# zhenghao2519/Beyond-Fixed-Forms

Hardware: AMD Instinct MI355X
Metric: scenes/sec (2D->3D projection+refinement), 200k pts x 300 views (higher is better)
Workload: dtype f64

## Files before the change

### beyond_fixed_forms_amd/_lib.py

```python
from __future__ import annotations

import ctypes
import os
import time
from ctypes import c_double, c_float, c_int32, c_int64, c_void_p

import torch

_HERE = os.path.dirname(os.path.abspath(__file__))
LIB_PATH = os.environ.get("BFF_HIP_LIB") or os.path.join(_HERE, "lib", "libbff_hip.so")
CSRC_DIR = os.path.join(_HERE, "csrc")

_P, _I, _L, _D, _F = c_void_p, c_int32, c_int64, c_double, c_float

SIGNATURES = {
    "bff_rle_to_maskbits": [_P, _P, _P, _P, _I, _L, _I, _P, _P, _P],
    "bff_rle_to_labels": [_P, _P, _P, _P, _I, _L, _I, _P, _P, _P, _P],
    "bff_mask_row_directory": [_P, _P, _P, _I, _I, _I, _P, _P],
    "bff_project_views_lookup": [_P, _L, _L, _P, _P, _I, _P, _I, _I, _I, _P, _I, _I, _D, _P, _P, _P, _P, _P, _I, _P, _P, _P, _P, _P, _L, _L, _P, _P, _P, _P],
    "bff_project_views_cached": [_L, _I, _P, _I, _I, _P, _P, _P, _P, _P, _P, _P, _P, _I, _P, _P, _P, _P, _P, _L, _L, _P, _P, _P, _P],
    "bff_visibility_table": [_P, _L, _L, _P, _P, _I, _P, _I, _I, _I, _I, _I, _D, _P, _P, _P, _P, _L, _P, _I, _P],
    "bff_visibility_sorted": [_P, _P, _P, _L, _L, _I, _I, _I, _P, _P, _P, _P, _P, _P],
    "bff_project_views_runs": [_L, _I, _P, _I, _I, _P, _P, _P, _P, _P, _P, _P, _P, _I, _P, _P, _P, _P, _P, _L, _L, _P, _P, _P, _P],
    "bff_masks2d_count": [_P, _I, _L, _P, _P, _P],
    "bff_masks2d_runs": [_P, _I, _L, _P, _P, _P, _P],
    "bff_project_views": [_P, _L, _L, _P, _P, _I, _P, _P, _I, _I, _D, _P, _P, _P, _I, _P, _P, _P, _P, _P, _L, _L, _P, _P, _P, _P, _P],
    "bff_depth_tile_u16": [_P, _I, _I, _I, _P, _I, _P],
    "bff_project_views_u16": [_P, _L, _L, _P, _P, _I, _P, _I, _I, _I, _P, _I, _I, _D, _P, _P, _P, _I, _P, _P, _P, _P, _P, _L, _L, _P, _P, _P, _P, _P],
    "bff_point_tile_bounds": [_P, _L, _L, _P, _P],
    "bff_count_viewed": [_P, _L, _L, _P, _P, _I, _P, _I, _I, _I, _P, _I, _I, _D, _I, _P, _P, _P],
    "bff_render_depth_u16": [_P, _L, _L, _P, _P, _I, _I, _I, _I, _I, _I, _P, _P, _P, _P],
    "bff_render_splat_depth_u16": [_P, _L, _L, _P, _P, _I, _I, _I, _I, _I, _D, _I, _P, _P, _P, _P],
    "bff_point_labels": [_P, _I, _L, _L, _P, _P, _P],
    "bff_render_labels_u16": [_P, _L, _L, _P, _P, _P, _I, _I, _I, _I, _I, _D, _I, _P, _P, _P, _P, _P],
    "bff_label_runs_count": [_P, _I, _I, _I, _I, _I, _I, _P, _P, _P],
    "bff_label_runs_emit": [_P, _I, _I, _I, _I, _I, _I, _P, _L, _P, _P, _P, _P],
    "bff_render_mesh_depth_u16": [_P, _L, _L, _P, _L, _P, _P, _I, _I, _I, _I, _I, _I, _P, _P, _P],
    "bff_render_mesh_depth_clip_u16": [_P, _L, _L, _P, _L, _P, _P, _I, _I, _I, _I, _I, _D, _I, _P, _P, _P],
# ... 392 lines not shown
def sweep_runs_ok(n_points):
    return bool(load().bff_sweep_runs_ok(n_points))


def project_views_runs(n_points, depth_index, height, width, vis, vis_sorted, run_start, run_end, mask_run_offs,
                       view_mask_offs, word_bits, frame_mask, frame_rowbase, frame_nmask, frame_flags, rows, masked_count,
                       viewed_count, chunk_mask):
    call("bff_project_views_runs", n_points, depth_index.shape[0], _ptr(depth_index, i32), height, width,
         _ptr(vis[0], i64), _ptr(vis_sorted[0], i32), _ptr(vis_sorted[1], i32), _ptr(vis_sorted[2], i32),
         _ptr(run_start, i32), _ptr(run_end, i32), _ptr(mask_run_offs, i32), _ptr(view_mask_offs, i32), word_bits,
         _ptr(frame_mask, i32), _ptr(frame_rowbase, i32), _ptr(frame_nmask, i32), _ptr(frame_flags, i32), _ptr(rows, i64),
         0 if rows is None else rows.shape[0], (n_points + 63) // 64, _ptr(chunk_mask, i64), _ptr(masked_count, i32),
         _ptr(viewed_count, i32))


def count_viewed(xyz_soa, n_points, inv_pose, cam_intr, depth, depth_index, height, width, depth_thresh, viewed_count,
                 tile_bounds=None, depth_size=None, frames_per_block=None):
    k = (c_double * 9)(*[float(v) for v in cam_intr.reshape(-1)])
    if depth.dtype == torch.int16 or depth_size is not None:
        hs, ws = (depth_size if depth_size is not None else depth.shape[1:3])
        layout = 0 if depth_size is None else (2 if depth.dtype == f32 else 1)
    else:
        hs, ws, layout = 0, 0, -1
        if depth.dtype != f32:
            raise TypeError(f"expected float32 depth images, got {depth.dtype}")
    if frames_per_block is None:
        frames_per_block = int(os.environ.get("BFF_VIEWED_TILE", "0"))
    call("bff_count_viewed", _ptr(xyz_soa, f64), n_points, xyz_soa.shape[1], _ptr(inv_pose, f64), ctypes.cast(k, c_void_p),
         inv_pose.shape[0], _ptr(depth), int(hs), int(ws), layout, _ptr(depth_index, i32), height, width,
         float(depth_thresh), int(frames_per_block), _ptr(viewed_count, i32), _ptr(tile_bounds, f64))
# ... 566 lines not shown
```

### beyond_fixed_forms_amd/csrc/common.h

```cpp
#pragma once

#include <hip/hip_runtime.h>

#include <cstdarg>
#include <cstdint>
#include <cstdio>

#include "bff_hip.h"

namespace bff {

constexpr int kWave = 64;
constexpr int kCW = 8;

char *err_buf();

inline int fail(int code, const char *fmt, ...) {
    va_list ap;
    va_start(ap, fmt);
    vsnprintf(err_buf(), 512, fmt, ap);
    va_end(ap);
    return code;
}

// ... 10 lines not shown
int &scratch_prezeroed();
inline hipError_t zero_async(void *p, size_t bytes, hipStream_t st)
{
    return scratch_prezeroed() ? hipSuccess : hipMemsetAsync(p, 0, bytes, st);
}

#define BFF_REQUIRE(cond, ...) \
    do { if (!(cond)) return ::bff::fail(BFF_E_ARG, __VA_ARGS__); } while (0)
#define BFF_LIMIT(cond, ...) \
    do { if (!(cond)) return ::bff::fail(BFF_E_LIMIT, __VA_ARGS__); } while (0)

__device__ __forceinline__ int lane_id() { return threadIdx.x & (kWave - 1); }

__device__ __forceinline__ int popc64(uint64_t v) { return __popcll(v); }

__device__ __forceinline__ void rle_word_edges(const uint64_t *row, int64_t w, int64_t nw, uint64_t &starts,
                                               uint64_t &ends)
{
    const uint64_t cur = w < nw ? row[w] : 0;
    const uint64_t prev_bit = w ? (row[w - 1] >> 63) : 0;
    const uint64_t shifted = (cur << 1) | prev_bit;
    starts = cur & ~shifted;
    ends = ~cur & shifted;
}

}
```

### beyond_fixed_forms_amd/csrc/merge.hip

```cpp
#include <hip/hip_ext.h>

#include <cstdlib>

#include "rows.h"

static thread_local hipEvent_t g_merge_start = nullptr, g_merge_stop = nullptr;

namespace bff {

constexpr int kBins = 64;

__device__ __forceinline__ int64_t heavy_signature(uint64_t heavy)
{
    uint32_t key = 0;
#pragma unroll
    for (int s = 0; s < 5; ++s) {
        int b = 63;
        if (heavy) { b = __ffsll((unsigned long long)heavy) - 1; heavy &= heavy - 1; }
        key = (key << 6) | (uint32_t)b;
    }
    return (int64_t)key;
}

__global__ __launch_bounds__(256) void row_stats_kernel(const uint64_t *__restrict__ rows, int64_t nw, int mw,
                                                         int bin_words, int32_t *__restrict__ area,
                                                         int32_t *__restrict__ mean_word,
                                                         uint64_t *__restrict__ cmask, uint32_t *__restrict__ hist,
                                                         int64_t *__restrict__ signature, uint16_t *__restrict__ cpop)
{
    extern __shared__ uint64_t s_cm[];
    __shared__ int part[4];
    __shared__ unsigned long long psum[4];
    __shared__ uint32_t s_hist[kBins];
    const int r = blockIdx.x, tid = threadIdx.x;
    const uint64_t *row = rows + (int64_t)r * nw;
    for (int i = tid; i < mw; i += 256) s_cm[i] = 0;
    if (tid < kBins) s_hist[tid] = 0;
// ... 1103 lines not shown
```

### beyond_fixed_forms_amd/csrc/project.hip

```cpp
#include <algorithm>
#include <cstdlib>

#include <hip/hip_ext.h>
#include <rocprim/device/device_radix_sort.hpp>

#include "common.h"
#include "mask_rows.h"

namespace bff {

constexpr int kBlock = 256;
constexpr int kPPT = 4;
constexpr int kWordsPerBlock = (kBlock / kWave) * kPPT;
constexpr int kPtsPerBlock = kWordsPerBlock * kWave;

struct Intrinsics { double k[9]; };

struct RawDepth {
    const uint32_t *taps;
    int n_taps;
    int texel_f32;
    int64_t frame_stride;
    float scale;
};
// ... 779 lines not shown
    const int64_t t = (int64_t)blockIdx.x * kBlock + threadIdx.x;
    if (t >= (int64_t)n_slots * (H + 1)) return;
    const int s = (int)(t / (H + 1)), y = (int)(t - (int64_t)s * (H + 1));
    int64_t lo = min((int64_t)off[s * stride], n_pairs);
    int64_t hi = s + 1 < n_slots ? min((int64_t)off[(s + 1) * stride], n_pairs) : n_pairs;
    const uint32_t target = (uint32_t)y * (uint32_t)W;
    while (lo < hi) {
        const int64_t mid = lo + ((hi - lo) >> 1);
        if (spix[mid] < target) lo = mid + 1; else hi = mid;
    }
    rowstart[t] = (uint32_t)lo;
}

constexpr int kRunsDeal = 4;

__global__ __launch_bounds__(kBlock) void sweep_runs_fill_kernel(
    int n_frames, const int32_t *__restrict__ depth_index, int H, int W,
    const uint32_t *__restrict__ spix, const uint32_t *__restrict__ spt, const uint32_t *__restrict__ rowstart,
    const int32_t *__restrict__ run_start, const int32_t *__restrict__ run_end, const int32_t *__restrict__ mask_run_offs,
    const int32_t *__restrict__ view_mask_offs, const int32_t *__restrict__ frame_mask,
    const int32_t *__restrict__ frame_rowbase, const int32_t *__restrict__ frame_nmask,
    uint64_t *__restrict__ rows, int64_t nw, int n_chunks, uint64_t *__restrict__ chunk_mask, int mw)
{
    extern __shared__ uint64_t s_row[];
    const int f = blockIdx.x, m = blockIdx.y;
    const int mi = frame_mask[f];
    if (mi < 0 || m >= frame_nmask[f]) return;
    const int tid = threadIdx.x, lane = tid & 63, wave = tid >> 6;
    const int64_t row = (int64_t)frame_rowbase[f] + m;
    for (int i = tid; i < n_chunks * kCW; i += kBlock) s_row[i] = 0;
    __syncthreads();

    const int g = view_mask_offs[mi] + m;
    const int r0 = mask_run_offs[g], r1 = mask_run_offs[g + 1];
    const uint32_t *rs = rowstart + (int64_t)depth_index[f] * (H + 1);
    const int hw = H * W;
    uint32_t *bits = reinterpret_cast<uint32_t *>(s_row);
    for (int rb = r0 + wave * kWave; rb < r1; rb += kBlock) {
        const int r = rb + lane;
        uint32_t lo = 0, cnt = 0;
        if (r < r1) {
            const int start = max(run_start[r], 0), end = min(run_end[r], hw);
            if (start < end) {
                const int y = start / W, ye = (end - 1) / W;
                uint32_t lo1 = rs[y], hi1 = rs[y + 1], lo2 = rs[ye], hi2 = rs[ye + 1];
// ... 48 lines not shown
        for (int h = 0; h < kCW; h += kPPT) {
            uint64_t o = 0;
#pragma unroll
            for (int q = 0; q < kPPT; ++q) o |= v[h + q];
            if (o) {
                any = true;
#pragma unroll
                for (int q = 0; q < kPPT; ++q) {
                    const int64_t w = (int64_t)c * kCW + h + q;
                    if (w < nw) rows[row * nw + w] = v[h + q];
                }
            }
        }
        const uint64_t flags = __ballot(any);
        if (lane == 0 && flags) chunk_mask[row * mw + (c0 >> 6)] |= flags;
    }
}

constexpr int kCountBlock = 1024;
constexpr int kCountBatch = 4;
constexpr int kCountList = 4096;

__global__ __launch_bounds__(kCountBlock) void sweep_runs_count_kernel(const uint64_t *__restrict__ rows, int64_t n_rows, int64_t nw,
                                                                       const uint64_t *__restrict__ chunk_mask, int mw,
                                                                       int64_t n_points, int32_t *__restrict__ masked_count)
{
    __shared__ int s_cnt[kCW * kWave];
    __shared__ int s_list[kCountList];
    __shared__ int s_n;
    const int tid = threadIdx.x, lane = tid & 63, wave = tid >> 6;
// ... 694 lines not shown

static int64_t runs_row_bytes(int64_t n_points)
{
    return (int64_t)sizeof(uint64_t) * kCW * ceil_div(ceil_div(n_points, (int64_t)kWave), (int64_t)kCW);
}

extern "C" int32_t bff_sweep_runs_ok(int64_t n_points)
{
    const char *on = getenv("BFF_SWEEP_RUNS"), *cap = getenv("BFF_SWEEP_RUNS_LDS_BYTES");
    if (on && on[0] == '0' && on[1] == 0) return 0;
    int64_t bound = kRunsLdsMax;
    if (cap && *cap) bound = std::min<int64_t>(bound, std::max<int64_t>(0, atoll(cap)));
    return n_points > 0 && runs_row_bytes(n_points) <= bound;
}

extern "C" int bff_project_views_runs(int64_t n_points, int32_t n_frames, const int32_t *depth_index, int32_t height,
                                      int32_t width, const uint64_t *vis_mask, const uint32_t *vis_spix,
                                      const uint32_t *vis_spt, const uint32_t *vis_rowstart, const int32_t *run_start,
                                      const int32_t *run_end, const int32_t *mask_run_offs, const int32_t *view_mask_offs,
                                      int32_t word_bits, const int32_t *frame_mask, const int32_t *frame_rowbase,
                                      const int32_t *frame_nmask, const int32_t *frame_flags, uint64_t *rows, int64_t n_rows,
                                      int64_t nw, uint64_t *chunk_mask, int32_t *masked_count, int32_t *viewed_count,
                                      void *stream)
{
    if (n_points <= 0 || n_frames <= 0) return BFF_OK;
    BFF_REQUIRE(height > 0 && width > 0, "bff_project_views_runs: bad image size");
    BFF_LIMIT((int64_t)height * width < (1ll << 31), "bff_project_views_runs: image larger than 2^31 pixels");
    BFF_REQUIRE(vis_mask && vis_spix && vis_spt && vis_rowstart, "bff_project_views_runs: null table");
    BFF_REQUIRE(word_bits == 32 || word_bits == 64, "bff_project_views_runs: word_bits must be 32 or 64");
    BFF_REQUIRE(depth_index && frame_mask && frame_rowbase && frame_nmask && frame_flags && run_start && run_end &&
                mask_run_offs && view_mask_offs && rows && chunk_mask && n_rows >= 0, "bff_project_views_runs: null pointer");
    BFF_REQUIRE(nw == ceil_div(n_points, 64), "bff_project_views_runs: nw must be ceil(n_points/64)");
    const int64_t row_bytes = runs_row_bytes(n_points);
    BFF_LIMIT(row_bytes <= kRunsLdsMax, "bff_project_views_runs: an instance row exceeds 64 KB of LDS (bff_sweep_runs_ok)");
    hipStream_t st = as_stream(stream);
    const int n_chunks = (int)ceil_div(nw, kCW), mw = (int)ceil_div(n_chunks, 64);
    const hipEvent_t ev0 = g_sweep_start, ev1 = g_sweep_stop;
    g_sweep_start = g_sweep_stop = nullptr;
    const bool count = masked_count != nullptr && n_rows > 0, viewed = viewed_count != nullptr;
    hipExtLaunchKernelGGL(sweep_runs_fill_kernel, dim3((unsigned)n_frames, (unsigned)word_bits), dim3(kBlock),
        (unsigned)row_bytes, st, ev0, (count || viewed) ? nullptr : ev1, 0,
        n_frames, depth_index, height, width, vis_spix, vis_spt, vis_rowstart, run_start, run_end, mask_run_offs,
        view_mask_offs, frame_mask, frame_rowbase, frame_nmask, rows, nw, n_chunks, chunk_mask, mw);
    if (count)
        hipExtLaunchKernelGGL(sweep_runs_count_kernel, dim3((unsigned)n_chunks), dim3(kCountBlock), 0, st,
            nullptr, viewed ? nullptr : ev1, 0, rows, n_rows, nw, chunk_mask, mw, n_points, masked_count);
    if (viewed)
        hipExtLaunchKernelGGL(sweep_runs_viewed_kernel, dim3((unsigned)ceil_div(nw, kBlock / kWave)), dim3(kBlock), 0, st,
            nullptr, ev1, 0, n_frames, depth_index, frame_flags, vis_mask, bff_visibility_words(n_points), nw, n_points,
            viewed_count);
    return launched("bff_project_views_runs");
}

extern "C" int bff_visibility_sorted_bytes(int32_t n_slots, int32_t height, int64_t n_pixels, int64_t *bytes)
{
    BFF_REQUIRE(n_slots >= 0 && height >= 0 && n_pixels >= 0 && bytes, "bff_visibility_sorted_bytes: bad arguments");
    bytes[0] = (int64_t)sizeof(uint32_t) * n_pixels;
    bytes[1] = (int64_t)sizeof(uint32_t) * n_pixels;
    bytes[2] = (int64_t)sizeof(uint32_t) * n_slots * ((int64_t)height + 1);
    return BFF_OK;
}

extern "C" int bff_visibility_sorted(const uint64_t *vis_mask, const uint32_t *vis_off, const uint32_t *vis_pix,
                                     int64_t n_pixels, int64_t n_points, int32_t n_slots, int32_t height, int32_t width,
                                     uint32_t *vis_spix, uint32_t *vis_spt, uint32_t *vis_rowstart, void *temp,
                                     size_t *temp_bytes, void *stream)
// ... 177 lines not shown
```

### beyond_fixed_forms_amd/csrc/scene.hip

```cpp
#include "rows.h"

using namespace bff;

namespace {

__global__ void order_keys_kernel(const int64_t *__restrict__ sig, const int32_t *__restrict__ label_id, int n,
                                  int sig_bits, int64_t *__restrict__ keys)
{
    const int i = blockIdx.x * blockDim.x + threadIdx.x;
    if (i < n) keys[i] = ((int64_t)label_id[i] << sig_bits) | sig[i];
}

int bits_for(int n)
{
    int b = 1;
    while ((1 << b) < n && b < 31) ++b;
    return b;
}

}

#define BFF_TRY(call) do { const int rc_ = (call); if (rc_ != BFF_OK) return rc_; } while (0)

extern "C" int32_t bff_scene_header_words(int32_t s1_rows, int32_t cap)
// ... 66 lines not shown
        BFF_TRY(hand_over(ws->events[0], stream, hv));
    }
    const bool cached = lookup && sc->vis_mask && sc->vis_off && sc->vis_pix;
    const bool runs = cached && sc->vis_spix && sc->vis_spt && sc->vis_rowstart && bff_sweep_runs_ok(n) != 0;
    if (lookup && !runs) {
        BFF_REQUIRE(ws->mask_tab && ws->mask_dir, "bff_scene_project: no row directory buffers");
        BFF_TRY(bff_mask_row_directory(sc->run_start, sc->run_end, sc->mask_run_offs, n_rows, sc->height, sc->width,
                                       ws->mask_tab, ws->mask_dir, hv));
    } else if (!lookup) {
        BFF_TRY(bff_rle_to_labels(sc->run_start, sc->run_end, sc->mask_run_offs, sc->view_mask_offs, sc->n_mviews, hw,
                                  sc->word_bits, ws->labels, ws->maskbits, ws->segmap, hv));
    }
    const bool ratio = pr->filter_mode == 2;
    int32_t *const sweep_viewed = (ratio && !viewed_in) ? ws->viewed : nullptr;
    const int32_t *const viewed = ratio ? (viewed_in ? viewed_in : ws->viewed) : nullptr;
    if (runs)
        BFF_TRY(bff_project_views_runs(n, sc->n_frames, sc->depth_index, sc->height, sc->width, sc->vis_mask, sc->vis_spix,
                                       sc->vis_spt, sc->vis_rowstart, sc->run_start, sc->run_end, sc->mask_run_offs,
                                       sc->view_mask_offs, sc->word_bits, sc->frame_mask, sc->frame_rowbase, sc->frame_nmask,
                                       sc->frame_flags, ws->rows, n_rows, nw, ws->chunk_mask, ws->masked, sweep_viewed, hv));
    else if (cached)
        BFF_TRY(bff_project_views_cached(n, sc->n_frames, sc->depth_index, sc->height, sc->width, sc->vis_mask, sc->vis_off,
                                         sc->vis_pix, ws->mask_tab, ws->mask_dir, sc->run_start, sc->run_end,
                                         sc->view_mask_offs, sc->word_bits, sc->frame_mask, sc->frame_rowbase, sc->frame_nmask,
                                         sc->frame_flags, ws->rows, n_rows, nw, ws->chunk_mask, ws->masked, sweep_viewed, hv));
    else if (lookup)
        BFF_TRY(bff_project_views_lookup(sc->xyz, n, sc->n_pad, sc->inv_pose, sc->cam_intr, sc->n_frames,
                                         sc->depth_raw ? sc->depth_raw : (const void *)sc->depth, sc->depth_h, sc->depth_w,
                                         sc->depth_raw ? sc->depth_tiled : -1, sc->depth_index, sc->height, sc->width,
                                         pr->depth_thresh, ws->mask_tab, ws->mask_dir, sc->run_start, sc->run_end,
                                         sc->view_mask_offs, sc->word_bits, sc->frame_mask, sc->frame_rowbase, sc->frame_nmask,
                                         sc->frame_flags, ws->rows, n_rows, nw, ws->chunk_mask, ws->masked, sweep_viewed,
                                         sc->tile_bounds, hv));
    else if (sc->depth_raw)
        BFF_TRY(bff_project_views_u16(sc->xyz, n, sc->n_pad, sc->inv_pose, sc->cam_intr, sc->n_frames, sc->depth_raw,
// ... 24 lines not shown
        } else {
            BFF_TRY(bff_point_threshold_pairs(ws->masked, viewed, n, pr->filter_fraction,
                                              ws->pair_scratch, reinterpret_cast<float *>(hdr + BFF_HDR_THR),
                                              hdr + BFF_HDR_NUNIQUE, hdr + BFF_HDR_OVERFLOW, stream));
        }
        BFF_TRY(bff_ratio_keep(ws->masked, viewed, n, 0.0f,
                               reinterpret_cast<const float *>(hdr + BFF_HDR_THR), 1, nw, ws->keep, stream));
    } else {
        BFF_TRY(bff_ratio_keep(ws->masked, nullptr, n, 0.0f, nullptr, 0, nw, ws->keep, stream));
    }
    if (fork) {
        hipError_t ee = hipEventRecord(reinterpret_cast<hipEvent_t>(ws->aux_events[1]), as_stream(stream));
        if (ee != hipSuccess) return fail((int)ee, "bff_scene_project: aux stream: %s", hipGetErrorString(ee));
        stream = main_stream;
    }
    uint16_t *cpop = bff_merge_uses_chunk_bound(nw) ? ws->chunk_pop : nullptr;
    BFF_TRY(bff_row_stats(ws->rows, n_rows, nw, ws->area, ws->mean_word, ws->chunk_mask, 1, ws->hist, ws->sig, cpop, stream));
    {
        const int64_t *keys = ws->sig;
        int key_bits = BFF_SIGNATURE_BITS;
        if (sc->n_label_ids > 1) {
            key_bits += bits_for(sc->n_label_ids);
            order_keys_kernel<<<(unsigned)ceil_div(n_rows, 256), 256, 0, st>>>(ws->sig, sc->label_id, n_rows,
                                                                              BFF_SIGNATURE_BITS, ws->sig_keys);
            keys = ws->sig_keys;
        }
        size_t tb = ws->sort_temp_bytes;
        BFF_TRY(bff_argsort_i64(keys, ws->sig_sorted, ws->order, n_rows, key_bits, ws->sort_temp, &tb, stream));
    }
    BFF_TRY(merge_components_streams(ws->rows, n_rows, nw, ws->order, n_rows, ws->chunk_mask, ws->tile_mask, ws->hist,
                                     ws->merge_scratch, ws->area, sc->label_id, pr->iou_thres, ws->parent, 1, nullptr, nullptr,
                                     cpop, stream, hv, ws->events[2], ws->events[3]));
// ... 32 lines not shown
```

### beyond_fixed_forms_amd/projection.py

```python
from __future__ import annotations

import dataclasses
from typing import List, Optional

import numpy as np
import torch

import os

from . import _lib, pipeline
from .scene import (DEPTH_THRESH, DeviceScene, prepare_class, prepare_geometry, prepare_scene,
                    with_viewed_counts)
from .timing import merge_span, span, sweep_span


@dataclasses.dataclass
class Stage2Result:
    scene_id: str
    n_points: int
    rows: torch.Tensor
    conf: torch.Tensor
    final_class: List[str]
    groups: list
    debug: dict
# ... 126 lines not shown
def fast_path_ok(ds: DeviceScene) -> bool:
    return (ds.n_rows > 0 and ds.n_points > 0 and ds.view_mask_offs.shape[0] > 1 and ds.n_mask_frames > 0
            and ds.xyz.is_cuda and os.environ.get("BFF_NO_FAST") != "1")


@dataclasses.dataclass
class VisibilityTable:
    mask: torch.Tensor
    off: torch.Tensor
    pix: torch.Tensor
    ready: torch.cuda.Event
    streams: set
    spix: Optional[torch.Tensor] = None
    spt: Optional[torch.Tensor] = None
    rowstart: Optional[torch.Tensor] = None

    def tensors(self):
        return [t for t in (self.mask, self.off, self.pix, self.spix, self.spt, self.rowstart) if t is not None]


def vis_table_max_bytes():
    return int(float(os.environ.get("BFF_VIS_TABLE_MAX_MB", "512")) * (1 << 20))


def scene_visibility(ds: DeviceScene, depth_thresh) -> Optional[VisibilityTable]:
    if os.environ.get("BFF_VIS_TABLE", "1") == "0" or not _lib.mask_lookup_rows(ds.height, ds.width, ds.n_rows):
        return None
    owner = ds.geometry if ds.geometry is not None else ds
    tables = owner.__dict__.setdefault("_vis_tables", {})
    key = float(depth_thresh)
    tab = tables.get(key)
    if tab is None:
        tables[key] = "visited"
        return None
    if tab is False:
        return None
    raw = _lib.raw_stream()
    if tab == "visited":
        dev = ds.xyz.device
        if ds.geometry is not None:
# ... 4 lines not shown
            slots, idx = np.unique(di, return_index=True)
            first[slots] = idx
            poses = ds.inv_pose[torch.as_tensor(first).to(dev)].contiguous()
        got = _lib.visibility_table(ds.xyz, ds.n_points, poses, ds.cam_intr, ds.sweep_depth, ds.height, ds.width, key,
                                    ds.tile_bounds, depth_size=ds.depth_size, max_bytes=vis_table_max_bytes(), with_count=True)
        if got is None:
            tables[key] = False
            return None
        got, n_pairs = got[:3], got[3]
        n_slots = int(got[0].shape[0])
        total = sum(_lib.visibility_table_bytes(ds.n_points, n_slots, n_pairs)) + \
            sum(_lib.visibility_sorted_bytes(n_slots, ds.height, n_pairs))
        companion = (None, None, None)
        if _lib.sweep_runs_ok(ds.n_points) and total <= vis_table_max_bytes() and n_slots * ds.height * ds.width <= 1 << 32:
            companion = _lib.visibility_sorted(got, n_pairs, ds.n_points, ds.height, ds.width)
        ready = torch.cuda.Event()
        ready.record(torch.cuda.current_stream(dev))
        tab = tables[key] = VisibilityTable(*got, ready, {raw}, *companion)
    elif raw not in tab.streams:
        st = torch.cuda.current_stream(ds.xyz.device)
        st.wait_event(tab.ready)
        for t in tab.tensors():
            t.record_stream(st)
        tab.streams.add(raw)
    return tab


def projection_front(ds: DeviceScene, cfg, debug_out: bool = False, timers=None, stage1=None, fast=None) -> _Front:
    if fast is None:
        fast = not debug_out
    do_ratio = with_viewed_counts(cfg)
    viewed_in = ds.viewed_in if do_ratio else None
    if do_ratio and ds.geometry is not None and viewed_in is None:
        raise ValueError("a class scene needs its geometry's viewed counts for the detection-ratio filter "
                         "(prepare the geometry with with_viewed=True)")
    if fast and fast_path_ok(ds) and (stage1 is None or stage1.n_points == ds.n_points):
        fr = _Front(ds, cfg, {}, False, do_ratio=do_ratio, stage1=stage1)
        vis = scene_visibility(ds, DEPTH_THRESH)
        fr.dbg["sweep"] = "plain" if vis is None else "cached"
        if vis is not None:
            fr.dbg["sweep_form"] = "runs" if vis.spix is not None and _lib.sweep_runs_ok(ds.n_points) else "points"
        with sweep_span(timers, "project_views"), merge_span(timers, "merge_components"):
            fr.fast = pipeline.issue(ds, cfg, DEPTH_THRESH, stage1,
                                     ds.n_frames if (do_ratio and viewed_in is None) else ds.n_mask_frames, viewed_in, vis)
        return fr
    with _lib.launch_stream():
        fr = _projection_front(ds, cfg, debug_out, timers, viewed_in=viewed_in)
        fr.stage1 = stage1
        return fr


def _projection_front(ds, cfg, debug_out, timers, viewed_in=None) -> _Front:
    dev = ds.xyz.device
    fr = _Front(ds, cfg, {}, debug_out)
    n, nw = ds.n_points, ds.nw
    do_ratio = fr.do_ratio = with_viewed_counts(cfg)

    n_mviews = ds.view_mask_offs.shape[0] - 1
    maskbits = torch.empty((n_mviews, ds.height * ds.width), device=dev,
# ... 74 lines not shown
    HDR_SIZES, HDR_FIRST, HDR_BEFORE, HDR_AFTER, HDR_CONF, HDR_CROSS = hdr_offsets(GROUP_CAP)
    dev = ds.xyz.device
    n, nw = ds.n_points, ds.nw
    k_all, flags = int(hdr[HDR_K]), int(hdr[HDR_K + 1])
    filtered = h["params"].filter_mode != 0
    if filtered:
        thr = float(hdr[HDR_THR:HDR_THR + 1].view(np.float32)[0])
        if hdr[HDR_NUNIQUE] == 0 or np.isnan(thr):
            ws.rows_dirty = True
            raise IndexError("index out of range: unique()[floor(t * n)] (P:516 / P:574)")
        dbg["thr"] = thr
    if flags:
        mw = max(_lib.load().bff_chunk_mask_words(nw), 1)
        hd = ws.t["hdr"]
        slow = _Front(ds, cfg, dbg, False, rows=ws.view("rows", ds.n_rows, nw), masked=ws.view("masked", n),
                      viewed=(ds.viewed_in if ds.viewed_in is not None else ws.view("viewed", n)) if fr.do_ratio else None,
                      keep=ws.view("keep", nw),
                      thr_dev=hd[HDR_THR:HDR_THR + 1].view(torch.float32) if filtered else None,
                      lat_info=hd[HDR_NUNIQUE:HDR_NUNIQUE + 1] if filtered else None,
                      area=ws.view("area", ds.n_rows), comp=ws.view("comp", ds.n_rows),
                      cmask=ws.view("chunk_mask", ds.n_rows, mw), arena=_WsRows(ws), do_ratio=fr.do_ratio)
        dbg["path"] = "general (device tables incomplete: %d groups, flags %d)" % (k_all, flags)
        return _projection_back(slow, None, None, stage1 if (stage1 is not None and stage1.n_points == n) else None)
    dbg["path"] = "fast"
    k = k_all
    if k == 0:
        dbg["groups"] = []
        return _empty(ds, dbg)
    sizes = hdr[HDR_SIZES:HDR_SIZES + k]
    first = hdr[HDR_FIRST:HDR_FIRST + k]
    before, after = hdr[HDR_BEFORE:HDR_BEFORE + k], hdr[HDR_AFTER:HDR_AFTER + k]
# ... 195 lines not shown
```

### include/bff_hip.h

```cpp
#ifndef BFF_HIP_H
#define BFF_HIP_H

#include <stddef.h>
#include <stdint.h>

#ifdef __cplusplus
extern "C" {
#endif

#define BFF_OK 0
#define BFF_E_ARG (-1)
#define BFF_E_LIMIT (-2)

#define BFF_ABI_VERSION 16

int bff_abi_version(void);
const char *bff_last_error(void);
const char *bff_arch(void);

int bff_host_component_csr(const int32_t *comp, const uint8_t *has_self_loop, int32_t n, int32_t min_members,
                           int32_t *offs, int32_t *members, int32_t *sizes, int32_t *n_void);

int bff_rle_to_maskbits(const int32_t *run_start, const int32_t *run_end, const int32_t *mask_run_offs,
                        const int32_t *view_mask_offs, int32_t n_views, int64_t n_pixels, int32_t word_bits,
// ... 246 lines not shown
                             int32_t *masked_count, int32_t *viewed_count, void *stream);

int bff_visibility_sorted(const uint64_t *vis_mask, const uint32_t *vis_off, const uint32_t *vis_pix, int64_t n_pixels,
                          int64_t n_points, int32_t n_slots, int32_t height, int32_t width, uint32_t *vis_spix,
                          uint32_t *vis_spt, uint32_t *vis_rowstart, void *temp, size_t *temp_bytes, void *stream);
int bff_visibility_sorted_bytes(int32_t n_slots, int32_t height, int64_t n_pixels, int64_t *bytes);

int32_t bff_sweep_runs_ok(int64_t n_points);
int bff_project_views_runs(int64_t n_points, int32_t n_frames, const int32_t *depth_index, int32_t height, int32_t width,
                           const uint64_t *vis_mask, const uint32_t *vis_spix, const uint32_t *vis_spt,
                           const uint32_t *vis_rowstart, const int32_t *run_start, const int32_t *run_end,
                           const int32_t *mask_run_offs, const int32_t *view_mask_offs, int32_t word_bits,
                           const int32_t *frame_mask, const int32_t *frame_rowbase, const int32_t *frame_nmask,
                           const int32_t *frame_flags, uint64_t *rows, int64_t n_rows, int64_t nw, uint64_t *chunk_mask,
                           int32_t *masked_count, int32_t *viewed_count, void *stream);

typedef struct bff_scene {
    int64_t n_points, n_pad, nw;
    const double *xyz;
    const double *tile_bounds;
    const double *inv_pose;
    double cam_intr[9];
    const float *depth;
    const void *depth_raw;
    const int32_t *depth_index, *frame_mask, *frame_rowbase, *frame_nmask, *frame_flags;
    const int32_t *run_start, *run_end, *mask_run_offs, *view_mask_offs;
    const void *conf;
    const int32_t *label_id;
    const int32_t *unsort;
    const int32_t *perm;
// ... 133 lines not shown
```

Measured before the change: 1549.

## Fuse row statistics into runs sweep kernel and cache per-point viewed counts

Computes the per-row area, mean word, 64-bin histogram, heavy-bin signature and chunk popcounts inside the runs-form sweep fill kernel using shared-memory atomics. This lets the scene path skip the separate row_stats pass over the mask rows. It also computes the viewed counts once when the visibility table is built, so the ratio filter can reuse them instead of redoing the viewed pass every call. The cost is extra shared atomics and register pressure in the sweep kernel, plus another cached tensor in the visibility table.

```diff
diff --git a/beyond_fixed_forms_amd/_lib.py b/beyond_fixed_forms_amd/_lib.py
--- a/beyond_fixed_forms_amd/_lib.py
+++ b/beyond_fixed_forms_amd/_lib.py
@@ -22,6 +22,9 @@
     "bff_visibility_table": [_P, _L, _L, _P, _P, _I, _P, _I, _I, _I, _I, _I, _D, _P, _P, _P, _P, _L, _P, _I, _P],
     "bff_visibility_sorted": [_P, _P, _P, _L, _L, _I, _I, _I, _P, _P, _P, _P, _P, _P],
     "bff_project_views_runs": [_L, _I, _P, _I, _I, _P, _P, _P, _P, _P, _P, _P, _P, _I, _P, _P, _P, _P, _P, _L, _L, _P, _P, _P, _P],
+    "bff_project_views_runs_stats": [_L, _I, _P, _I, _I, _P, _P, _P, _P, _P, _P, _P, _P, _I, _P, _P, _P, _P, _P, _L, _L, _P, _P,
+                                     _P, _P, _P, _P, _P, _P, _P],
+    "bff_visibility_viewed": [_L, _I, _P, _P, _P, _P, _P],
     "bff_masks2d_count": [_P, _I, _L, _P, _P, _P],
     "bff_masks2d_runs": [_P, _I, _L, _P, _P, _P, _P],
     "bff_project_views": [_P, _L, _L, _P, _P, _I, _P, _P, _I, _I, _D, _P, _P, _P, _I, _P, _P, _P, _P, _P, _L, _L, _P, _P, _P, _P, _P],
@@ -444,6 +447,33 @@
          _ptr(viewed_count, i32))
 
 
+def project_views_runs_stats(n_points, depth_index, height, width, vis, vis_sorted, run_start, run_end, mask_run_offs,
+                             view_mask_offs, word_bits, frame_mask, frame_rowbase, frame_nmask, frame_flags, rows,
+                             masked_count, viewed_count, chunk_mask, with_chunk_pop=True):
+    n = rows.shape[0]
+    dev = rows.device
+    area = torch.zeros(n, dtype=i32, device=dev)
+    mean_word = torch.zeros(n, dtype=i32, device=dev)
+    hist = torch.zeros((n, 64), dtype=i32, device=dev)
+    sig = torch.zeros(n, dtype=i64, device=dev)
+    cpop = torch.empty((n, chunk_mask.shape[1] * 64), dtype=torch.int16, device=dev) if with_chunk_pop else None
+    call("bff_project_views_runs_stats", n_points, depth_index.shape[0], _ptr(depth_index, i32), height, width,
+         _ptr(vis[0], i64), _ptr(vis_sorted[0], i32), _ptr(vis_sorted[1], i32), _ptr(vis_sorted[2], i32),
+         _ptr(run_start, i32), _ptr(run_end, i32), _ptr(mask_run_offs, i32), _ptr(view_mask_offs, i32), word_bits,
+         _ptr(frame_mask, i32), _ptr(frame_rowbase, i32), _ptr(frame_nmask, i32), _ptr(frame_flags, i32), _ptr(rows, i64),
+         n, (n_points + 63) // 64, _ptr(chunk_mask, i64), _ptr(masked_count, i32), _ptr(viewed_count, i32), _ptr(area),
+         _ptr(mean_word), _ptr(hist), _ptr(sig), _ptr(cpop))
+    hist.chunk_pop = cpop
+    return area, mean_word, chunk_mask, hist, sig
+
+
+def visibility_viewed(n_points, depth_index, frame_flags, vis_mask):
+    viewed = torch.zeros(max(n_points, 1), dtype=i32, device=vis_mask.device)[:n_points]
+    call("bff_visibility_viewed", n_points, depth_index.shape[0], _ptr(depth_index, i32), _ptr(frame_flags, i32),
+         _ptr(vis_mask, i64), _ptr(viewed, i32))
+    return viewed
+
+
 def count_viewed(xyz_soa, n_points, inv_pose, cam_intr, depth, depth_index, height, width, depth_thresh, viewed_count,
                  tile_bounds=None, depth_size=None, frames_per_block=None):
     k = (c_double * 9)(*[float(v) for v in cam_intr.reshape(-1)])
diff --git a/beyond_fixed_forms_amd/csrc/common.h b/beyond_fixed_forms_amd/csrc/common.h
--- a/beyond_fixed_forms_amd/csrc/common.h
+++ b/beyond_fixed_forms_amd/csrc/common.h
@@ -48,6 +48,20 @@
 
 __device__ __forceinline__ int popc64(uint64_t v) { return __popcll(v); }
 
+constexpr int kBins = 64;
+
+__device__ __forceinline__ int64_t heavy_signature(uint64_t heavy)
+{
+    uint32_t key = 0;
+#pragma unroll
+    for (int s = 0; s < 5; ++s) {
+        int b = 63;
+        if (heavy) { b = __ffsll((unsigned long long)heavy) - 1; heavy &= heavy - 1; }
+        key = (key << 6) | (uint32_t)b;
+    }
+    return (int64_t)key;
+}
+
 __device__ __forceinline__ void rle_word_edges(const uint64_t *row, int64_t w, int64_t nw, uint64_t &starts,
                                                uint64_t &ends)
 {
diff --git a/beyond_fixed_forms_amd/csrc/merge.hip b/beyond_fixed_forms_amd/csrc/merge.hip
--- a/beyond_fixed_forms_amd/csrc/merge.hip
+++ b/beyond_fixed_forms_amd/csrc/merge.hip
@@ -8,19 +8,6 @@
 
 namespace bff {
 
-constexpr int kBins = 64;
-
-__device__ __forceinline__ int64_t heavy_signature(uint64_t heavy)
-{
-    uint32_t key = 0;
-#pragma unroll
-    for (int s = 0; s < 5; ++s) {
-        int b = 63;
-        if (heavy) { b = __ffsll((unsigned long long)heavy) - 1; heavy &= heavy - 1; }
-        key = (key << 6) | (uint32_t)b;
-    }
-    return (int64_t)key;
-}
 
 __global__ __launch_bounds__(256) void row_stats_kernel(const uint64_t *__restrict__ rows, int64_t nw, int mw,
                                                          int bin_words, int32_t *__restrict__ area,
diff --git a/beyond_fixed_forms_amd/csrc/project.hip b/beyond_fixed_forms_amd/csrc/project.hip
--- a/beyond_fixed_forms_amd/csrc/project.hip
+++ b/beyond_fixed_forms_amd/csrc/project.hip
@@ -817,21 +817,34 @@
 
 constexpr int kRunsDeal = 4;
 
+struct RunsStats {
+    int32_t *area, *mean_word;
+    uint32_t *hist;
+    int64_t *signature;
+    uint16_t *cpop;
+    int bin_words;
+};
+
+template <bool kStats>
 __global__ __launch_bounds__(kBlock) void sweep_runs_fill_kernel(
     int n_frames, const int32_t *__restrict__ depth_index, int H, int W,
     const uint32_t *__restrict__ spix, const uint32_t *__restrict__ spt, const uint32_t *__restrict__ rowstart,
     const int32_t *__restrict__ run_start, const int32_t *__restrict__ run_end, const int32_t *__restrict__ mask_run_offs,
     const int32_t *__restrict__ view_mask_offs, const int32_t *__restrict__ frame_mask,
     const int32_t *__restrict__ frame_rowbase, const int32_t *__restrict__ frame_nmask,
-    uint64_t *__restrict__ rows, int64_t nw, int n_chunks, uint64_t *__restrict__ chunk_mask, int mw)
+    uint64_t *__restrict__ rows, int64_t nw, int n_chunks, uint64_t *__restrict__ chunk_mask, int mw, RunsStats st)
 {
     extern __shared__ uint64_t s_row[];
+    __shared__ uint32_t s_hist[kStats ? kBins : 1];
+    __shared__ unsigned long long s_wsum;
     const int f = blockIdx.x, m = blockIdx.y;
     const int mi = frame_mask[f];
     if (mi < 0 || m >= frame_nmask[f]) return;
     const int tid = threadIdx.x, lane = tid & 63, wave = tid >> 6;
     const int64_t row = (int64_t)frame_rowbase[f] + m;
     for (int i = tid; i < n_chunks * kCW; i += kBlock) s_row[i] = 0;
+    if (kStats && tid < kBins) s_hist[tid] = 0;
+    if (kStats && tid == 0) s_wsum = 0;
     __syncthreads();
 
     const int g = view_mask_offs[mi] + m;
@@ -910,6 +923,49 @@
         }
         const uint64_t flags = __ballot(any);
         if (lane == 0 && flags) chunk_mask[row * mw + (c0 >> 6)] |= flags;
+        if (kStats && any) {
+            int pc[kCW], in_chunk = 0, weighted = 0;
+#pragma unroll
+            for (int q = 0; q < kCW; ++q) {
+                pc[q] = popc64(v[q]);
+                in_chunk += pc[q];
+                weighted += q * pc[q];
+            }
+            const int w0 = c * kCW;
+            int bin = w0 / st.bin_words;
+            int left = (bin + 1) * st.bin_words - w0;
+            uint32_t in_bin = 0;
+#pragma unroll
+            for (int q = 0; q < kCW; ++q) {
+                if (left == 0) {
+                    if (in_bin) atomicAdd(&s_hist[bin], in_bin);
+                    ++bin;
+                    left = st.bin_words;
+                    in_bin = 0;
+                }
+                in_bin += (uint32_t)pc[q];
+                --left;
+            }
+            if (in_bin) atomicAdd(&s_hist[bin], in_bin);
+            atomicAdd(&s_wsum, (unsigned long long)((uint32_t)w0 * (uint32_t)in_chunk + (uint32_t)weighted));
+            if (st.cpop) st.cpop[row * mw * 64 + c] = (uint16_t)in_chunk;
+        }
+    }
+    if (kStats) {
+        __syncthreads();
+        if (tid < kBins) {
+            const uint32_t hv = s_hist[tid];
+            int a = (int)hv;
+#pragma unroll
+            for (int d = 32; d > 0; d >>= 1) a += __shfl_xor(a, d);
+            st.hist[row * kBins + tid] = hv;
+            const uint64_t heavy = __ballot((uint64_t)hv * 100 >= (uint64_t)a * 15 && a > 0);
+            if (tid == 0) {
+                st.signature[row] = heavy_signature(a ? heavy : 0);
+                st.area[row] = a;
+                st.mean_word[row] = a ? (int32_t)(s_wsum / (unsigned long long)a) : 0x7fffffff;
+            }
+        }
     }
 }
 
@@ -1634,14 +1690,14 @@
     return n_points > 0 && runs_row_bytes(n_points) <= bound;
 }
 
-extern "C" int bff_project_views_runs(int64_t n_points, int32_t n_frames, const int32_t *depth_index, int32_t height,
-                                      int32_t width, const uint64_t *vis_mask, const uint32_t *vis_spix,
-                                      const uint32_t *vis_spt, const uint32_t *vis_rowstart, const int32_t *run_start,
-                                      const int32_t *run_end, const int32_t *mask_run_offs, const int32_t *view_mask_offs,
-                                      int32_t word_bits, const int32_t *frame_mask, const int32_t *frame_rowbase,
-                                      const int32_t *frame_nmask, const int32_t *frame_flags, uint64_t *rows, int64_t n_rows,
-                                      int64_t nw, uint64_t *chunk_mask, int32_t *masked_count, int32_t *viewed_count,
-                                      void *stream)
+static int project_views_runs_launch(int64_t n_points, int32_t n_frames, const int32_t *depth_index, int32_t height,
+                                     int32_t width, const uint64_t *vis_mask, const uint32_t *vis_spix,
+                                     const uint32_t *vis_spt, const uint32_t *vis_rowstart, const int32_t *run_start,
+                                     const int32_t *run_end, const int32_t *mask_run_offs, const int32_t *view_mask_offs,
+                                     int32_t word_bits, const int32_t *frame_mask, const int32_t *frame_rowbase,
+                                     const int32_t *frame_nmask, const int32_t *frame_flags, uint64_t *rows, int64_t n_rows,
+                                     int64_t nw, uint64_t *chunk_mask, int32_t *masked_count, int32_t *viewed_count,
+                                     const RunsStats *stats, void *stream)
 {
     if (n_points <= 0 || n_frames <= 0) return BFF_OK;
     BFF_REQUIRE(height > 0 && width > 0, "bff_project_views_runs: bad image size");
@@ -1658,10 +1714,14 @@
     const hipEvent_t ev0 = g_sweep_start, ev1 = g_sweep_stop;
     g_sweep_start = g_sweep_stop = nullptr;
     const bool count = masked_count != nullptr && n_rows > 0, viewed = viewed_count != nullptr;
-    hipExtLaunchKernelGGL(sweep_runs_fill_kernel, dim3((unsigned)n_frames, (unsigned)word_bits), dim3(kBlock),
-        (unsigned)row_bytes, st, ev0, (count || viewed) ? nullptr : ev1, 0,
-        n_frames, depth_index, height, width, vis_spix, vis_spt, vis_rowstart, run_start, run_end, mask_run_offs,
-        view_mask_offs, frame_mask, frame_rowbase, frame_nmask, rows, nw, n_chunks, chunk_mask, mw);
+    static_assert(kBins == kWave, "sweep_runs_fill_kernel: one histogram bin per lane of its first wave");
+#define BFF_RUNS_FILL(STATS, ARG)                                                                                         \
+    hipExtLaunchKernelGGL(sweep_runs_fill_kernel<STATS>, dim3((unsigned)n_frames, (unsigned)word_bits), dim3(kBlock),    \
+        (unsigned)row_bytes, st, ev0, (count || viewed) ? nullptr : ev1, 0,                                              \
+        n_frames, depth_index, height, width, vis_spix, vis_spt, vis_rowstart, run_start, run_end, mask_run_offs,        \
+        view_mask_offs, frame_mask, frame_rowbase, frame_nmask, rows, nw, n_chunks, chunk_mask, mw, ARG)
+    if (stats) { BFF_RUNS_FILL(true, *stats); } else { BFF_RUNS_FILL(false, RunsStats{}); }
+#undef BFF_RUNS_FILL
     if (count)
         hipExtLaunchKernelGGL(sweep_runs_count_kernel, dim3((unsigned)n_chunks), dim3(kCountBlock), 0, st,
             nullptr, viewed ? nullptr : ev1, 0, rows, n_rows, nw, chunk_mask, mw, n_points, masked_count);
@@ -1670,6 +1730,58 @@
             nullptr, ev1, 0, n_frames, depth_index, frame_flags, vis_mask, bff_visibility_words(n_points), nw, n_points,
             viewed_count);
     return launched("bff_project_views_runs");
+}
+
+extern "C" int bff_project_views_runs(int64_t n_points, int32_t n_frames, const int32_t *depth_index, int32_t height,
+                                      int32_t width, const uint64_t *vis_mask, const uint32_t *vis_spix,
+                                      const uint32_t *vis_spt, const uint32_t *vis_rowstart, const int32_t *run_start,
+                                      const int32_t *run_end, const int32_t *mask_run_offs, const int32_t *view_mask_offs,
+                                      int32_t word_bits, const int32_t *frame_mask, const int32_t *frame_rowbase,
+                                      const int32_t *frame_nmask, const int32_t *frame_flags, uint64_t *rows, int64_t n_rows,
+                                      int64_t nw, uint64_t *chunk_mask, int32_t *masked_count, int32_t *viewed_count,
+                                      void *stream)
+{
+    return project_views_runs_launch(n_points, n_frames, depth_index, height, width, vis_mask, vis_spix, vis_spt, vis_rowstart,
+                                     run_start, run_end, mask_run_offs, view_mask_offs, word_bits, frame_mask, frame_rowbase,
+                                     frame_nmask, frame_flags, rows, n_rows, nw, chunk_mask, masked_count, viewed_count,
+                                     nullptr, stream);
+}
+
+extern "C" int bff_project_views_runs_stats(int64_t n_points, int32_t n_frames, const int32_t *depth_index, int32_t height,
+                                            int32_t width, const uint64_t *vis_mask, const uint32_t *vis_spix,
+                                            const uint32_t *vis_spt, const uint32_t *vis_rowstart, const int32_t *run_start,
+                                            const int32_t *run_end, const int32_t *mask_run_offs,
+                                            const int32_t *view_mask_offs, int32_t word_bits, const int32_t *frame_mask,
+                                            const int32_t *frame_rowbase, const int32_t *frame_nmask,
+                                            const int32_t *frame_flags, uint64_t *rows, int64_t n_rows, int64_t nw,
+                                            uint64_t *chunk_mask, int32_t *masked_count, int32_t *viewed_count, int32_t *area,
+                                            int32_t *mean_word, uint32_t *hist, int64_t *signature, uint16_t *chunk_pop,
+                                            void *stream)
+{
+    if (n_points <= 0 || n_frames <= 0) return BFF_OK;
+    BFF_REQUIRE(area && mean_word && hist && signature, "bff_project_views_runs_stats: null pointer");
+    BFF_REQUIRE(n_rows >= 0 && nw == ceil_div(n_points, 64), "bff_project_views_runs_stats: bad sizes");
+    if (chunk_pop && n_rows > 0) {
+        const int64_t mw = ceil_div(ceil_div(nw, kCW), 64);
+        hipError_t e = zero_async(chunk_pop, sizeof(uint16_t) * (size_t)n_rows * mw * 64, as_stream(stream));
+        if (e != hipSuccess) return fail((int)e, "bff_project_views_runs_stats: memset: %s", hipGetErrorString(e));
+    }
+    const RunsStats stats{area, mean_word, hist, signature, chunk_pop, (int)ceil_div(nw, kBins)};
+    return project_views_runs_launch(n_points, n_frames, depth_index, height, width, vis_mask, vis_spix, vis_spt, vis_rowstart,
+                                     run_start, run_end, mask_run_offs, view_mask_offs, word_bits, frame_mask, frame_rowbase,
+                                     frame_nmask, frame_flags, rows, n_rows, nw, chunk_mask, masked_count, viewed_count,
+                                     &stats, stream);
+}
+
+extern "C" int bff_visibility_viewed(int64_t n_points, int32_t n_frames, const int32_t *depth_index,
+                                     const int32_t *frame_flags, const uint64_t *vis_mask, int32_t *viewed_count, void *stream)
+{
+    if (n_points <= 0 || n_frames <= 0) return BFF_OK;
+    BFF_REQUIRE(depth_index && frame_flags && vis_mask && viewed_count, "bff_visibility_viewed: null pointer");
+    const int64_t nw = ceil_div(n_points, 64);
+    sweep_runs_viewed_kernel<<<(unsigned)ceil_div(nw, kBlock / kWave), kBlock, 0, as_stream(stream)>>>(
+        n_frames, depth_index, frame_flags, vis_mask, bff_visibility_words(n_points), nw, n_points, viewed_count);
+    return launched("bff_visibility_viewed");
 }
 
 extern "C" int bff_visibility_sorted_bytes(int32_t n_slots, int32_t height, int64_t n_pixels, int64_t *bytes)
diff --git a/beyond_fixed_forms_amd/csrc/scene.hip b/beyond_fixed_forms_amd/csrc/scene.hip
--- a/beyond_fixed_forms_amd/csrc/scene.hip
+++ b/beyond_fixed_forms_amd/csrc/scene.hip
@@ -104,11 +104,13 @@
     const bool ratio = pr->filter_mode == 2;
     int32_t *const sweep_viewed = (ratio && !viewed_in) ? ws->viewed : nullptr;
     const int32_t *const viewed = ratio ? (viewed_in ? viewed_in : ws->viewed) : nullptr;
+    uint16_t *const cpop = bff_merge_uses_chunk_bound(nw) ? ws->chunk_pop : nullptr;
     if (runs)
-        BFF_TRY(bff_project_views_runs(n, sc->n_frames, sc->depth_index, sc->height, sc->width, sc->vis_mask, sc->vis_spix,
-                                       sc->vis_spt, sc->vis_rowstart, sc->run_start, sc->run_end, sc->mask_run_offs,
-                                       sc->view_mask_offs, sc->word_bits, sc->frame_mask, sc->frame_rowbase, sc->frame_nmask,
-                                       sc->frame_flags, ws->rows, n_rows, nw, ws->chunk_mask, ws->masked, sweep_viewed, hv));
+        BFF_TRY(bff_project_views_runs_stats(n, sc->n_frames, sc->depth_index, sc->height, sc->width, sc->vis_mask, sc->vis_spix,
+                                             sc->vis_spt, sc->vis_rowstart, sc->run_start, sc->run_end, sc->mask_run_offs,
+                                             sc->view_mask_offs, sc->word_bits, sc->frame_mask, sc->frame_rowbase,
+                                             sc->frame_nmask, sc->frame_flags, ws->rows, n_rows, nw, ws->chunk_mask, ws->masked,
+                                             sweep_viewed, ws->area, ws->mean_word, ws->hist, ws->sig, cpop, hv));
     else if (cached)
         BFF_TRY(bff_project_views_cached(n, sc->n_frames, sc->depth_index, sc->height, sc->width, sc->vis_mask, sc->vis_off,
                                          sc->vis_pix, ws->mask_tab, ws->mask_dir, sc->run_start, sc->run_end,
@@ -163,8 +165,8 @@
         if (ee != hipSuccess) return fail((int)ee, "bff_scene_project: aux stream: %s", hipGetErrorString(ee));
         stream = main_stream;
     }
-    uint16_t *cpop = bff_merge_uses_chunk_bound(nw) ? ws->chunk_pop : nullptr;
-    BFF_TRY(bff_row_stats(ws->rows, n_rows, nw, ws->area, ws->mean_word, ws->chunk_mask, 1, ws->hist, ws->sig, cpop, stream));
+    if (!runs)
+        BFF_TRY(bff_row_stats(ws->rows, n_rows, nw, ws->area, ws->mean_word, ws->chunk_mask, 1, ws->hist, ws->sig, cpop, stream));
     {
         const int64_t *keys = ws->sig;
         int key_bits = BFF_SIGNATURE_BITS;
diff --git a/beyond_fixed_forms_amd/projection.py b/beyond_fixed_forms_amd/projection.py
--- a/beyond_fixed_forms_amd/projection.py
+++ b/beyond_fixed_forms_amd/projection.py
@@ -164,16 +164,17 @@
     spix: Optional[torch.Tensor] = None
     spt: Optional[torch.Tensor] = None
     rowstart: Optional[torch.Tensor] = None
+    viewed: Optional[torch.Tensor] = None
 
     def tensors(self):
-        return [t for t in (self.mask, self.off, self.pix, self.spix, self.spt, self.rowstart) if t is not None]
+        return [t for t in (self.mask, self.off, self.pix, self.spix, self.spt, self.rowstart, self.viewed) if t is not None]
 
 
 def vis_table_max_bytes():
     return int(float(os.environ.get("BFF_VIS_TABLE_MAX_MB", "512")) * (1 << 20))
 
 
-def scene_visibility(ds: DeviceScene, depth_thresh) -> Optional[VisibilityTable]:
+def scene_visibility(ds: DeviceScene, depth_thresh, with_viewed: bool = False) -> Optional[VisibilityTable]:
     if os.environ.get("BFF_VIS_TABLE", "1") == "0" or not _lib.mask_lookup_rows(ds.height, ds.width, ds.n_rows):
         return None
     owner = ds.geometry if ds.geometry is not None else ds
@@ -208,9 +209,12 @@
         companion = (None, None, None)
         if _lib.sweep_runs_ok(ds.n_points) and total <= vis_table_max_bytes() and n_slots * ds.height * ds.width <= 1 << 32:
             companion = _lib.visibility_sorted(got, n_pairs, ds.n_points, ds.height, ds.width)
+        viewed = None
+        if with_viewed and ds.geometry is None and companion[0] is not None and ds.n_viewed > 0:
+            viewed = _lib.visibility_viewed(ds.n_points, ds.depth_index[:ds.n_frames], ds.frame_flags[:ds.n_frames], got[0])
         ready = torch.cuda.Event()
         ready.record(torch.cuda.current_stream(dev))
-        tab = tables[key] = VisibilityTable(*got, ready, {raw}, *companion)
+        tab = tables[key] = VisibilityTable(*got, ready, {raw}, *companion, viewed)
     elif raw not in tab.streams:
         st = torch.cuda.current_stream(ds.xyz.device)
         st.wait_event(tab.ready)
@@ -230,13 +234,18 @@
                          "(prepare the geometry with with_viewed=True)")
     if fast and fast_path_ok(ds) and (stage1 is None or stage1.n_points == ds.n_points):
         fr = _Front(ds, cfg, {}, False, do_ratio=do_ratio, stage1=stage1)
-        vis = scene_visibility(ds, DEPTH_THRESH)
+        vis = scene_visibility(ds, DEPTH_THRESH, with_viewed=do_ratio)
         fr.dbg["sweep"] = "plain" if vis is None else "cached"
         if vis is not None:
             fr.dbg["sweep_form"] = "runs" if vis.spix is not None and _lib.sweep_runs_ok(ds.n_points) else "points"
+        n_frames = ds.n_frames if (do_ratio and viewed_in is None) else ds.n_mask_frames
+        if do_ratio:
+            fr.dbg["viewed_pass"] = "sweep" if viewed_in is None else "geometry"
+            if viewed_in is None and vis is not None and vis.viewed is not None and fr.dbg["sweep_form"] == "runs":
+                viewed_in = vis.viewed
+                fr.dbg["viewed_pass"] = "table"
         with sweep_span(timers, "project_views"), merge_span(timers, "merge_components"):
-            fr.fast = pipeline.issue(ds, cfg, DEPTH_THRESH, stage1,
-                                     ds.n_frames if (do_ratio and viewed_in is None) else ds.n_mask_frames, viewed_in, vis)
+            fr.fast = pipeline.issue(ds, cfg, DEPTH_THRESH, stage1, n_frames, viewed_in, vis)
         return fr
     with _lib.launch_stream():
         fr = _projection_front(ds, cfg, debug_out, timers, viewed_in=viewed_in)
@@ -341,7 +350,7 @@
         mw = max(_lib.load().bff_chunk_mask_words(nw), 1)
         hd = ws.t["hdr"]
         slow = _Front(ds, cfg, dbg, False, rows=ws.view("rows", ds.n_rows, nw), masked=ws.view("masked", n),
-                      viewed=(ds.viewed_in if ds.viewed_in is not None else ws.view("viewed", n)) if fr.do_ratio else None,
+                      viewed=(h["args"][5] if h["args"][5] is not None else ws.view("viewed", n)) if fr.do_ratio else None,
                       keep=ws.view("keep", nw),
                       thr_dev=hd[HDR_THR:HDR_THR + 1].view(torch.float32) if filtered else None,
                       lat_info=hd[HDR_NUNIQUE:HDR_NUNIQUE + 1] if filtered else None,
diff --git a/include/bff_hip.h b/include/bff_hip.h
--- a/include/bff_hip.h
+++ b/include/bff_hip.h
@@ -284,6 +284,16 @@
                            const int32_t *frame_mask, const int32_t *frame_rowbase, const int32_t *frame_nmask,
                            const int32_t *frame_flags, uint64_t *rows, int64_t n_rows, int64_t nw, uint64_t *chunk_mask,
                            int32_t *masked_count, int32_t *viewed_count, void *stream);
+int bff_project_views_runs_stats(int64_t n_points, int32_t n_frames, const int32_t *depth_index, int32_t height,
+                                 int32_t width, const uint64_t *vis_mask, const uint32_t *vis_spix, const uint32_t *vis_spt,
+                                 const uint32_t *vis_rowstart, const int32_t *run_start, const int32_t *run_end,
+                                 const int32_t *mask_run_offs, const int32_t *view_mask_offs, int32_t word_bits,
+                                 const int32_t *frame_mask, const int32_t *frame_rowbase, const int32_t *frame_nmask,
+                                 const int32_t *frame_flags, uint64_t *rows, int64_t n_rows, int64_t nw,
+                                 uint64_t *chunk_mask, int32_t *masked_count, int32_t *viewed_count, int32_t *area,
+                                 int32_t *mean_word, uint32_t *hist, int64_t *signature, uint16_t *chunk_pop, void *stream);
+int bff_visibility_viewed(int64_t n_points, int32_t n_frames, const int32_t *depth_index, const int32_t *frame_flags,
+                          const uint64_t *vis_mask, int32_t *viewed_count, void *stream);
 
 typedef struct bff_scene {
     int64_t n_points, n_pad, nw;
```

Result: slower. 1489 (-3.9%).
